# Tai-Wang/Depth-from-Motion

Hardware: NVIDIA H100
Metric: frames/sec (higher is better)
Workload: dtype f32 (bf16x2 split operands, fp32 accumulate)

## Files before the change

### depth_from_motion_b200/csrc/conv_tc.cuh

```cuda
#pragma once
#include <cuda.h>
#include <cuda_bf16.h>

#include <algorithm>
#include <cstdlib>
#include <type_traits>
#include <vector>

#include "common.cuh"
#include "simt_kernels.cuh"
#include "wgmma.cuh"

namespace dfm {

inline uint16_t bf16_rn_bits(float f) {
  uint32_t u;
  memcpy(&u, &f, 4);
  if ((u & 0x7F800000u) == 0x7F800000u) return (uint16_t)(u >> 16);
  u += 0x7FFFu + ((u >> 16) & 1u);
  return (uint16_t)(u >> 16);
}
inline float bf16_bits_to_float(uint16_t b) {
  uint32_t u = (uint32_t)b << 16;
  float f;
  memcpy(&f, &u, 4);
  return f;
}

inline int tc_sm_count() {
  int& cached = per_device<int, 1>();
  if (!cached) cudaDeviceGetAttribute(&cached, cudaDevAttrMultiProcessorCount, cur_device());
  return cached;
}

enum { TC_S1 = 0, TC_S2 = 1, TC_T = 2 };
constexpr int TC_BX = 8, TC_BY = 16;
constexpr int TC_MMA_THREADS = 256;
constexpr int TC_LOAD_THREADS = 256;
constexpr int TC_THREADS = TC_MMA_THREADS + TC_LOAD_THREADS;
constexpr int TC_MAXOPS = 9, TC_MAXBLK = 48;
constexpr int TC_ZERO_TAP = 255;

template <int MODE>
struct TcMode;
template <>
struct TcMode<TC_S1> {
  static constexpr int PXB = 10, PYB = 18, PITCH = 10, ROWS = 186, CG = 32, NSTAGE = 4;
  static constexpr int SLOT_BLOCKS = 1;
  __host__ __device__ static int zo_of(int zi, int dz) { return zi + dz; }
  __host__ __device__ static int zi_first(int zo) { return zo - 1; }
  __host__ __device__ static int zi_last(int zo) { return zo + 1; }
  __host__ __device__ static int ptype(int) { return 0; }
};
template <>
struct TcMode<TC_S2> {
  static constexpr int PXB = 17, PYB = 33, PITCH = 9, ROWS = 620, CG = 16, NSTAGE = 3;
  static constexpr int SLOT_BLOCKS = 1;
  __host__ __device__ static int zo_of(int zi, int dz) { return (zi >> 1) + dz; }
  __host__ __device__ static int zi_first(int zo) { return 2 * zo - 1; }
  __host__ __device__ static int zi_last(int zo) { return 2 * zo + 1; }
  __host__ __device__ static int ptype(int zi) { return zi & 1; }
};
template <>
struct TcMode<TC_T> {
  static constexpr int PXB = 9, PYB = 17, PITCH = 9, ROWS = 154, CG = 32, NSTAGE = 4;
  static constexpr int SLOT_BLOCKS = 4;
  __host__ __device__ static int zo_of(int zi, int dz) { return 2 * zi + dz; }
  __host__ __device__ static int zi_first(int zo) { return zo >> 1; }
  __host__ __device__ static int zi_last(int zo) { return (zo + 1) >> 1; }
  __host__ __device__ static int ptype(int) { return 0; }
};

inline int tc_mode_of(const ConvGeom& g) {
  if (g.transposed) return TC_T;
  if (g.sd == 1 && g.sh == 1 && g.sw == 1 && g.pd == 1 && g.ph == 1 && g.pw == 1) return TC_S1;
  if (g.sd == 2 && g.sh == 2 && g.sw == 2 && g.pd == 1 && g.ph == 1 && g.pw == 1 &&
      g.Di % 2 == 0 && g.Hi % 2 == 0 && g.Wi % 2 == 0)
    return TC_S2;
  return -1;
}
inline bool tc_supported(int Cin, int Cout, int ) {
  if (Cin != 32 && Cin != 64) return false;
  const int ncta = 1024 / Cin;
  return Cout % ncta == 0 && Cout <= 64;
}
inline bool tc_geom_supported(const ConvGeom& g) { return tc_mode_of(g) >= 0; }

struct TcOp {
  uint32_t a_off;
  uint32_t b_off;
  uint32_t b_lbo;
  uint16_t blk0, blk1;
  uint32_t nruns;
  uint32_t runs[3];
};
struct TcBlk {
  int8_t dz;
  uint8_t colblk;
  uint8_t tap;
  uint8_t pad;
};
struct TcProgram {
  int nops;
  uint32_t need;
  TcOp ops[TC_MAXOPS];
  TcBlk blks[TC_MAXBLK];
};

template <int MODE>
inline void tc_build_program(int ptype, int Cin, int ncta, uint32_t* w_cursor, TcProgram* pr) {
  using M = TcMode<MODE>;
  pr->nops = 0;
  pr->need = 0;
  int nb = 0;
  auto add_op = [&](int a_rows, std::vector<TcBlk> blks) {
    TcOp& op = pr->ops[pr->nops++];
    op.a_off = (uint32_t)a_rows * 16;
    op.b_off = *w_cursor;
    op.b_lbo = (uint32_t)blks.size() * ncta * 16;
    op.blk0 = (uint16_t)nb;
    for (TcBlk b : blks) pr->blks[nb++] = b;
    op.blk1 = (uint16_t)nb;
    *w_cursor += (uint32_t)(Cin / 8) * op.b_lbo;
    op.nruns = 0;
    size_t i = 0;
    while (i < blks.size()) {
      size_t e = i + 1;
      auto lin = [&](const TcBlk& b) { return (b.dz + 1) * M::SLOT_BLOCKS + b.colblk; };
      while (e < blks.size() && lin(blks[e]) == lin(blks[i]) + (int)(e - i)) ++e;
      const int nblk = (int)(e - i);
      op.runs[op.nruns++] = (uint32_t)nblk | ((uint32_t)i << 4) | ((uint32_t)lin(blks[i]) << 10);
      for (size_t k = i; k < e; ++k) pr->need |= 1u << (blks[k].dz + 1);
      i = e;
    }
  };
  if (MODE == TC_S1) {
    for (int t = 0; t < 9; ++t) {
      const int dy = t / 3, dx = t % 3;
      add_op(dy * M::PITCH + dx, {TcBlk{-1, 0, (uint8_t)(18 + t), 0}, TcBlk{0, 0, (uint8_t)(9 + t), 0},
                                  TcBlk{1, 0, (uint8_t)t, 0}});
    }
  } else if (MODE == TC_S2) {
    for (int t = 0; t < 9; ++t) {
      const int dy = t / 3, dx = t % 3;
      const int a_rows = (((dx & 1) * 2 + (dy & 1)) * 17 + (dy >> 1)) * M::PITCH + (dx >> 1);
      if (ptype == 0)
        add_op(a_rows, {TcBlk{0, 0, (uint8_t)(9 + t), 0}});
      else
        add_op(a_rows, {TcBlk{0, 0, (uint8_t)(18 + t), 0}, TcBlk{1, 0, (uint8_t)t, 0}});
    }
  } else {
    const int cls_px[4] = {0, 1, 1, 0}, cls_py[4] = {0, 0, 1, 1};
    for (int sh = 0; sh < 4; ++sh) {
      const int sx = sh & 1, sy = sh >> 1;
      std::vector<TcBlk> blks;
      for (int dz = -1; dz <= 1; ++dz) {
        const int kz = dz + 1;
        for (int c = 0; c < 4; ++c) {
          const int px = cls_px[c], py = cls_py[c];
          int kx = -1, ky = -1;
          if (px == 0) { if (!sx) kx = 1; } else kx = sx ? 0 : 2;
          if (py == 0) { if (!sy) ky = 1; } else ky = sy ? 0 : 2;
          const bool real = kx >= 0 && ky >= 0;
          blks.push_back(TcBlk{(int8_t)dz, (uint8_t)c,
                               (uint8_t)(real ? kz * 9 + ky * 3 + kx : TC_ZERO_TAP), 0});
        }
      }
      if (sh == 3) {
        std::vector<TcBlk> real;
        for (const TcBlk& b : blks)
          if (b.tap != TC_ZERO_TAP) real.push_back(b);
        blks = real;
      } else {
        while (!blks.empty() && blks.front().tap == TC_ZERO_TAP) blks.erase(blks.begin());
        while (!blks.empty() && blks.back().tap == TC_ZERO_TAP) blks.pop_back();
      }
      add_op(sy * M::PITCH + sx, blks);
    }
  }
}

struct TcWeights {
  uint8_t* dev = nullptr;
  int Cin = 0, Cout = 0, ncta = 0, nsplit = 0, mode = -1, kslice = 0;
  uint32_t image_bytes = 0, hi_bytes = 0;
  TcProgram prog[2];

  bool ready() const { return dev != nullptr; }
  void release() {
    if (dev) cudaFree(dev);
    dev = nullptr;
  }
  template <int MODE>
  bool build_mode(const float* packed, int cin, int cout, std::string* err, bool ks = false) {
    release();
    mode = MODE;
    Cin = cin;
    Cout = cout;
    kslice = ks ? 1 : 0;
    const int cin_img = ks ? 16 : cin;
    ncta = ks ? cout : 1024 / cin;
    nsplit = ks ? cin / 16 : cout / ncta;
    uint32_t cursor = 0;
    const int ntypes = MODE == TC_S2 ? 2 : 1;
    for (int t = 0; t < ntypes; ++t) tc_build_program<MODE>(t, cin_img, ncta, &cursor, &prog[t]);
    hi_bytes = cursor;
    image_bytes = 2 * hi_bytes;
    std::vector<uint16_t> img((size_t)nsplit * image_bytes / 2);
    const int kch = cin_img / 8;
    for (int s = 0; s < nsplit; ++s)
      for (int t = 0; t < ntypes; ++t)
        for (int o = 0; o < prog[t].nops; ++o) {
          const TcOp& op = prog[t].ops[o];
          const int nblk = op.blk1 - op.blk0;
          for (int kc = 0; kc < kch; ++kc)
            for (int b = 0; b < nblk; ++b)
              for (int j = 0; j < ncta; ++j)
                for (int e = 0; e < 8; ++e) {
                  const int tap = prog[t].blks[op.blk0 + b].tap;
                  if (tap == TC_ZERO_TAP) continue;
                  const int ci = kc * 8 + e + (ks ? s * 16 : 0), co = ks ? j : s * ncta + j;
                  const float w = packed[((size_t)tap * cin + ci) * cout + co];
                  const uint16_t hi = bf16_rn_bits(w);
                  const uint16_t lo = bf16_rn_bits(w - bf16_bits_to_float(hi));
                  const size_t off = (size_t)s * image_bytes / 2 + op.b_off / 2 +
                                     ((size_t)kc * nblk * ncta + (size_t)b * ncta + j) * 8 + e;
                  img[off] = hi;
                  img[off + hi_bytes / 2] = lo;
                }
        }
    if (cudaMalloc(&dev, img.size() * 2) != cudaSuccess ||
        cudaMemcpy(dev, img.data(), img.size() * 2, cudaMemcpyHostToDevice) != cudaSuccess) {
      if (err) *err = "TcWeights: device upload failed";
      release();
      return false;
    }
    return true;
  }
  bool build(const float* packed, int cin, int cout, int m, std::string* err) {
    static const bool no_ks1 = getenv("DFM_NO_KSLICE") != nullptr;
    static const bool ks1 = getenv("DFM_KSLICE_S1") != nullptr;
    if (m == TC_S1) return build_mode<TC_S1>(packed, cin, cout, err,
                                             cin == 64 && cout == 64 && !no_ks1 && ks1);
    if (m == TC_S2) {
      static const bool no_ks = getenv("DFM_NO_KSLICE") != nullptr;
      return build_mode<TC_S2>(packed, cin, cout, err, cout == 64 && !no_ks);
    }
    return build_mode<TC_T>(packed, cin, cout, err);
  }
};

__device__ __forceinline__ uint32_t smem_u32(const void* p) {
  return static_cast<uint32_t>(__cvta_generic_to_shared(p));
}
__device__ __forceinline__ void mbar_init(uint32_t bar, uint32_t count) {
  asm volatile("mbarrier.init.shared::cta.b64 [%0], %1;" ::"r"(bar), "r"(count));
}
__device__ __forceinline__ void mbar_arrive(uint32_t bar) {
  asm volatile("mbarrier.arrive.shared::cta.b64 _, [%0];" ::"r"(bar) : "memory");
}
__device__ __forceinline__ void mbar_wait(uint32_t bar, uint32_t parity, int* err) {
  for (int it = 0; it < (1 << 26); ++it) {
    uint32_t ok;
    asm volatile(
        "{\n\t.reg .pred q;\n\t"
        "mbarrier.try_wait.parity.shared::cta.b64 q, [%1], %2;\n\t"
        "selp.u32 %0, 1, 0, q;\n\t}\n"
        : "=r"(ok)
        : "r"(bar), "r"(parity)
        : "memory");
    if (ok) return;
  }
  *reinterpret_cast<volatile int*>(err) = 1;
  __threadfence_system();
}
__device__ __forceinline__ void mbar_wait_timed(uint32_t bar, uint32_t parity, int* err,
                                                unsigned long long& acc, bool timed) {
  if (!timed) {
    mbar_wait(bar, parity, err);
    return;
  }
  const long long t0 = clock64();
  mbar_wait(bar, parity, err);
  acc += (unsigned long long)(clock64() - t0);
}
__device__ __forceinline__ bool elect_one() {
  uint32_t pred;
  asm volatile(
      "{\n\t.reg .pred p;\n\telect.sync _|p, 0xffffffff;\n\tselp.u32 %0, 1, 0, p;\n\t}\n"
      : "=r"(pred));
  return pred != 0;
}
__device__ __forceinline__ void desc_add(uint64_t& d, uint32_t inc16) {
  asm("{\n\t.reg .b32 lo, hi;\n\tmov.b64 {lo, hi}, %0;\n\tadd.u32 lo, lo, %1;\n\t"
      "mov.b64 %0, {lo, hi};\n\t}\n"
      : "+l"(d)
      : "r"(inc16));
}
__device__ __forceinline__ uint64_t pack64(uint32_t lo, uint32_t hi) {
  return ((uint64_t)hi << 32) | lo;
}
__device__ __forceinline__ void split_store(const float v[8], uint8_t* hi_dst, uint8_t* lo_dst) {
  uint32_t h[4], l[4];
#pragma unroll
  for (int i = 0; i < 4; ++i) {
    const __nv_bfloat162 hh = __floats2bfloat162_rn(v[2 * i], v[2 * i + 1]);
    const float2 hf = __bfloat1622float2(hh);
    const __nv_bfloat162 ll = __floats2bfloat162_rn(v[2 * i] - hf.x, v[2 * i + 1] - hf.y);
    h[i] = *reinterpret_cast<const uint32_t*>(&hh);
    l[i] = *reinterpret_cast<const uint32_t*>(&ll);
  }
  *reinterpret_cast<uint4*>(hi_dst) = make_uint4(h[0], h[1], h[2], h[3]);
  *reinterpret_cast<uint4*>(lo_dst) = make_uint4(l[0], l[1], l[2], l[3]);
}

#ifndef DFM_LD_VARIANT
#define DFM_LD_VARIANT 0
#endif
__device__ __forceinline__ float4 ld_act(const float4* p) {
#if DFM_LD_VARIANT == 1
  return __ldcg(p);
#elif DFM_LD_VARIANT == 2
  float4 v;
  asm volatile("ld.global.nc.L1::no_allocate.L2::256B.v4.f32 {%0,%1,%2,%3}, [%4];"
               : "=f"(v.x), "=f"(v.y), "=f"(v.z), "=f"(v.w) : "l"(p));
  return v;
#elif DFM_LD_VARIANT == 3
  return __ldcs(p);
#elif DFM_LD_VARIANT == 4
  float4 v;
  asm volatile("ld.global.nc.L1::no_allocate.v4.f32 {%0,%1,%2,%3}, [%4];"
               : "=f"(v.x), "=f"(v.y), "=f"(v.z), "=f"(v.w) : "l"(p));
  return v;
#else
  return __ldg(p);
#endif
}

template <int NT>
struct SrcLoader8 {
  static constexpr bool kTma = false;
  Src s;
  int C, H, W;
  static constexpr int BATCH = 6 / NT;
  struct Raw {
    float4 a[NT][2];
  };
  __device__ __forceinline__ void issue(int z, int y, int x, int c0, Raw& r) const {
    const long long inpl = ((long long)y * W + x) * C + c0, plane = (long long)H * W * C;
#pragma unroll
    for (int t = 0; t < NT; ++t) {
      const float* px = s.t[t].x + term_plane(s.t[t], z) * plane + inpl;
      r.a[t][0] = ld_act(reinterpret_cast<const float4*>(px));
      r.a[t][1] = ld_act(reinterpret_cast<const float4*>(px) + 1);
    }
  }
  __device__ __forceinline__ void finish(const Raw& r, int c0, float v[8]) const {
#pragma unroll
    for (int i = 0; i < 8; ++i) v[i] = 0.f;
#pragma unroll
    for (int t = 0; t < NT; ++t) {
      {
        float u[8] = {r.a[t][0].x, r.a[t][0].y, r.a[t][0].z, r.a[t][0].w,
                      r.a[t][1].x, r.a[t][1].y, r.a[t][1].z, r.a[t][1].w};
        if (s.t[t].scale) {
          const float4 s0 = __ldg(reinterpret_cast<const float4*>(s.t[t].scale + c0));
          const float4 s1 = __ldg(reinterpret_cast<const float4*>(s.t[t].scale + c0) + 1);
          const float4 h0 = __ldg(reinterpret_cast<const float4*>(s.t[t].shift + c0));
          const float4 h1 = __ldg(reinterpret_cast<const float4*>(s.t[t].shift + c0) + 1);
          const float sc[8] = {s0.x, s0.y, s0.z, s0.w, s1.x, s1.y, s1.z, s1.w};
          const float sh[8] = {h0.x, h0.y, h0.z, h0.w, h1.x, h1.y, h1.z, h1.w};
#pragma unroll
          for (int i = 0; i < 8; ++i) u[i] = fmaf(u[i], sc[i], sh[i]);
        }
        if (s.t[t].relu) {
#pragma unroll
          for (int i = 0; i < 8; ++i) u[i] = fmaxf(u[i], 0.f);
        }
#pragma unroll
        for (int i = 0; i < 8; ++i) v[i] += u[i];
      }
    }
    if (s.outer_relu) {
#pragma unroll
      for (int i = 0; i < 8; ++i) v[i] = fmaxf(v[i], 0.f);
    }
  }
};

struct WarpLoader8 {
  static constexpr bool kTma = false;
  WarpLoader w;
  static constexpr int BATCH = 1;
  struct Raw {
    float4 t[4][2];
    float wt[4];
  };
  __device__ __forceinline__ void issue(int z, int y, int x, int c0, Raw& r) const {
    c0 += w.first;
    if (c0 < w.C) {
      const float* p = w.cur + ((long long)(y * w.g.step) * w.g.Wf + x * w.g.step) * w.C + c0;
      r.t[0][0] = __ldg(reinterpret_cast<const float4*>(p));
      r.t[0][1] = __ldg(reinterpret_cast<const float4*>(p) + 1);
      r.wt[0] = 1.f;
      r.wt[1] = r.wt[2] = r.wt[3] = 0.f;
      return;
    }
    c0 -= w.C;
    float fx, fy;
    warp_coord(w.g, x, y, __ldg(w.depths + z), fx, fy);
    const Taps t = bilinear_taps(fx, fy, w.g.Hf, w.g.Wf);
#pragma unroll
    for (int k = 0; k < 4; ++k) {
      r.wt[k] = t.w[k];
      if (t.w[k] != 0.f) {
        const float* p = w.prev + (long long)t.off[k] * w.C + c0;
        r.t[k][0] = __ldg(reinterpret_cast<const float4*>(p));
        r.t[k][1] = __ldg(reinterpret_cast<const float4*>(p) + 1);
      }
    }
  }
  __device__ __forceinline__ void finish(const Raw& r, int, float v[8]) const {
#pragma unroll
    for (int i = 0; i < 8; ++i) v[i] = 0.f;
#pragma unroll
    for (int k = 0; k < 4; ++k) {
      if (r.wt[k] != 0.f) {
        v[0] = fmaf(r.wt[k], r.t[k][0].x, v[0]); v[1] = fmaf(r.wt[k], r.t[k][0].y, v[1]);
        v[2] = fmaf(r.wt[k], r.t[k][0].z, v[2]); v[3] = fmaf(r.wt[k], r.t[k][0].w, v[3]);
        v[4] = fmaf(r.wt[k], r.t[k][1].x, v[4]); v[5] = fmaf(r.wt[k], r.t[k][1].y, v[5]);
        v[6] = fmaf(r.wt[k], r.t[k][1].z, v[6]); v[7] = fmaf(r.wt[k], r.t[k][1].w, v[7]);
      }
    }
  }
};

struct TmaLoader8 {
  static constexpr bool kTma = true;
  static constexpr int BATCH = 1;
  CUtensorMap map;
  int nch_total;
  struct Raw {};
  __device__ __forceinline__ void issue(int, int, int, int, Raw&) const {}
  __device__ __forceinline__ void finish(const Raw&, int, float v[8]) const {
#pragma unroll
    for (int i = 0; i < 8; ++i) v[i] = 0.f;
  }
};
constexpr int TMA_S2_CLS = 17 * 9;
constexpr int TMA_S2_CLSR = (2 * TMA_S2_CLS + 7) / 8 * 8;

__device__ __forceinline__ void tma_load_4d(uint32_t dst, const CUtensorMap* map, int c1, int c2,
                                            int c3, uint32_t bar) {
  asm volatile(
      "cp.async.bulk.tensor.4d.shared::cluster.global.tile.mbarrier::complete_tx::bytes "
      "[%0], [%1, {%2, %3, %4, %5}], [%6];" ::"r"(dst),
      "l"(map), "r"(0), "r"(c1), "r"(c2), "r"(c3), "r"(bar)
      : "memory");
}

constexpr int PS_XRUN = 64, PS_WARPS = 4, PS_SEG = 33;
inline size_t presplit_smem_bytes(int C) { return (size_t)PS_WARPS * 4 * (C / 8) * PS_SEG * 16; }
template <int NT>
__global__ void __launch_bounds__(32 * PS_WARPS)
presplit_kernel(const SrcLoader8<NT> ld, int Z, uint4* __restrict__ out) {
  extern __shared__ uint4 ps_sm[];
  const int nch = ld.C >> 3, W = ld.W, H = ld.H, W2 = W >> 1, H2 = H >> 1;
  const int warp = threadIdx.x >> 5, lane = threadIdx.x & 31;
  uint4* sm = ps_sm + (size_t)warp * 4 * nch * PS_SEG;
  const int runs_per_row = (W + PS_XRUN - 1) / PS_XRUN;
  const long long nruns = (long long)Z * H * runs_per_row;
  for (long long r = (long long)blockIdx.x * PS_WARPS + warp; r < nruns;
       r += (long long)gridDim.x * PS_WARPS) {
    const int run = (int)(r % runs_per_row);
    const long long zy = r / runs_per_row;
    const int y = (int)(zy % H), z = (int)(zy / H);
    const int xb = run * PS_XRUN;
#pragma unroll 4
    for (int i = lane; i < PS_XRUN * nch; i += 32) {
      const int xl = i / nch, chunk = i - xl * nch, x = xb + xl;
      if (x < W) {
        typename SrcLoader8<NT>::Raw raw;
        ld.issue(z, y, x, chunk * 8, raw);
        float val[8];
        ld.finish(raw, chunk * 8, val);
        uint4* hi = sm + ((xl & 1) * nch + chunk) * PS_SEG + (xl >> 1);
        split_store(val, reinterpret_cast<uint8_t*>(hi),
                    reinterpret_cast<uint8_t*>(hi + 2 * nch * PS_SEG));
      }
    }
    __syncwarp();
    const int py = y & 1, y2 = y >> 1, x2 = (xb >> 1) + lane;
    for (int seg = 0; seg < 4 * nch; ++seg) {
      const int chunk = seg % nch, px = (seg / nch) & 1, hl = seg / (2 * nch);
      if (2 * x2 + px < W)
        out[((((long long)(z * 2 + hl) * 4 + py * 2 + px) * nch + chunk) * H2 + y2) * W2 + x2] =
            sm[seg * PS_SEG + lane];
    }
    __syncwarp();
  }
}
inline bool presplit_launch(const Src& s, int C, int Z, int H, int W, uint4* out, cudaStream_t st) {
  if ((H | W) & 1) return false;
  const size_t smem = presplit_smem_bytes(C);
  const long long nruns = (long long)Z * H * ((W + PS_XRUN - 1) / PS_XRUN);
  const int blocks = (int)std::min<long long>((nruns + PS_WARPS - 1) / PS_WARPS, 12LL * tc_sm_count());
  auto go = [&](auto kern, auto ld) {
    if (cudaFuncSetAttribute(kern, cudaFuncAttributeMaxDynamicSharedMemorySize, (int)smem) !=
        cudaSuccess)
      return false;
    kern<<<blocks, 32 * PS_WARPS, smem, st>>>(ld, Z, out);
    return cudaGetLastError() == cudaSuccess;
  };
  if (s.n == 1) return go(presplit_kernel<1>, SrcLoader8<1>{s, C, H, W});
  if (s.n == 2) return go(presplit_kernel<2>, SrcLoader8<2>{s, C, H, W});
  return go(presplit_kernel<3>, SrcLoader8<3>{s, C, H, W});
}

inline bool make_presplit_map_s2(CUtensorMap* map, const void* base, int W, int H,
                                 long long slabs, std::string* err) {
  typedef CUresult (*EncodeFn)(CUtensorMap*, CUtensorMapDataType, cuuint32_t, void*,
                               const cuuint64_t*, const cuuint64_t*, const cuuint32_t*,
                               const cuuint32_t*, CUtensorMapInterleave, CUtensorMapSwizzle,
                               CUtensorMapL2promotion, CUtensorMapFloatOOBfill);
  static EncodeFn encode = nullptr;
  if (!encode) {
    void* fn = nullptr;
    cudaDriverEntryPointQueryResult qres;
    if (cudaGetDriverEntryPoint("cuTensorMapEncodeTiled", &fn, cudaEnableDefault, &qres) !=
            cudaSuccess || !fn || qres != cudaDriverEntryPointSuccess) {
      if (err) *err = "cuTensorMapEncodeTiled is not available from this driver";
      return false;
    }
    encode = (EncodeFn)fn;
  }
  const int W2 = W / 2, H2 = H / 2;
  const cuuint64_t dims[4] = {8, (cuuint64_t)W2, (cuuint64_t)H2, (cuuint64_t)slabs};
  const cuuint64_t strides[3] = {16, (cuuint64_t)W2 * 16, (cuuint64_t)H2 * W2 * 16};
  const cuuint32_t box[4] = {8, 9, 17, 2};
  const cuuint32_t estr[4] = {1, 1, 1, 1};
  const CUresult r = encode(map, CU_TENSOR_MAP_DATA_TYPE_UINT16, 4, const_cast<void*>(base), dims,
                            strides, box, estr, CU_TENSOR_MAP_INTERLEAVE_NONE,
                            CU_TENSOR_MAP_SWIZZLE_NONE, CU_TENSOR_MAP_L2_PROMOTION_L2_128B,
                            CU_TENSOR_MAP_FLOAT_OOB_FILL_NONE);
  if (r != CUDA_SUCCESS) {
    if (err) *err = "cuTensorMapEncodeTiled failed with code " + std::to_string((int)r);
    return false;
  }
  return true;
}

struct TcParams {
  const uint8_t* wimg;
  float* out;
  double* stats;
  int Di, Hi, Wi;
  int Do, Ho, Wo, Cout;
  int Mx, My;
  int tiles_x, tiles_y, nsplit;
  int z_unit;
  uint32_t w_bytes, w_hi_bytes;
  int* err;
  unsigned long long* role_cycles;
  const float* addend;
  int zw_lo, zw_hi;
  float zw;
  long long slice_stride;
  int store1;
  int dbg;
};

struct TcItem {
  int x0, y0, split, z_lo, z_hi;
};
struct TcWalk {
  long long cur, end;
  int split;
};
__device__ __forceinline__ TcWalk tc_walk_begin(const TcParams& p) {
  TcWalk w;
  const int per_split = gridDim.x / p.nsplit;
  w.split = blockIdx.x % p.nsplit;
  const int r = blockIdx.x / p.nsplit;
  const long long units_col = p.Do / p.z_unit;
  const long long total = (long long)p.tiles_x * p.tiles_y * units_col;
  w.cur = total * r / per_split;
  w.end = total * (r + 1) / per_split;
  return w;
}
__device__ __forceinline__ bool tc_walk_next(const TcParams& p, TcWalk& w, TcItem& it) {
  if (w.cur >= w.end) return false;
  const long long units_col = p.Do / p.z_unit;
  const int col = (int)(w.cur / units_col);
  const long long u0 = w.cur % units_col;
  const long long u1 = min(units_col, u0 + (w.end - w.cur));
  it.split = w.split;
  it.x0 = (col % p.tiles_x) * TC_BX;
  it.y0 = (col / p.tiles_x) * TC_BY;
  it.z_lo = (int)u0 * p.z_unit;
  it.z_hi = (int)u1 * p.z_unit;
  w.cur += u1 - u0;
  return true;
}

template <int MODE>
struct TcWin;
template <>
struct TcWin<TC_S1> {
  static constexpr int NPL = 3;
  __device__ static int base(int zi) { return zi - 1; }
};
template <>
struct TcWin<TC_S2> {
  static constexpr int NPL = 2;
  __device__ static int base(int zi) { return zi >> 1; }
};
template <>
struct TcWin<TC_T> {
  static constexpr int NPL = 3;
  __device__ static int base(int zi) { return 2 * zi - 1; }
};

template <int MODE, int CIN, int NCTA, class Loader>
__global__ void __launch_bounds__(TC_THREADS, 1) conv_tc_kernel(const __grid_constant__ TcParams p,
                                                                 const __grid_constant__ Loader ld) {
  using M = TcMode<MODE>;
  using Win = TcWin<MODE>;
  constexpr bool TMA = Loader::kTma;
  static_assert(!TMA || MODE == TC_S2, "the TMA loader serves the stride-2 brick only");
  constexpr int CG = M::CG < CIN ? M::CG : CIN;
  constexpr int NCH = CG / 8;
  constexpr int NCG = CIN / CG;
  static_assert(!TMA || NCH == 2, "TMA stride-2 stages hold two 8-channel chunks");
  constexpr uint32_t S2_CLS16 = TMA ? TMA_S2_CLSR : TMA_S2_CLS;
  constexpr uint32_t A_LBO = TMA ? TMA_S2_CLS * 16 : M::ROWS * 16;
  constexpr uint32_t A_SBO = M::PITCH * 16;
  constexpr uint32_t A_HL = TMA ? 4 * TMA_S2_CLSR * 16 : NCH * M::ROWS * 16;
  constexpr uint32_t STAGE_BYTES = 2 * A_HL;
  constexpr uint32_t B_SBO = 128;
  constexpr bool KSLICE = CIN == 16;
  constexpr int NPOS = M::PXB * M::PYB;
  constexpr int LGROUPS = 2;
  constexpr int LG_THREADS = TC_LOAD_THREADS / LGROUPS;
  constexpr int NITEM = (NPOS * NCH + LG_THREADS - 1) / LG_THREADS;
  constexpr int PCOLS = M::SLOT_BLOCKS * NCTA;
  constexpr int NACC = Win::NPL * PCOLS / 2;

  extern __shared__ __align__(1024) uint8_t smem[];
  uint8_t* w_s = smem;
  uint8_t* a_s = smem + p.w_bytes;
  uint64_t* bars = reinterpret_cast<uint64_t*>(a_s + M::NSTAGE * STAGE_BYTES);

  const int tid = threadIdx.x, lane = tid & 31;
  const int warp = __shfl_sync(0xffffffffu, tid >> 5, 0);
  const uint32_t bar0 = smem_u32(bars);
  auto full_a = [&](int s) { return bar0 + 8u * s; };
  auto empty_a = [&](int s) { return bar0 + 8u * (M::NSTAGE + s); };
  const uint32_t w_bar = bar0 + 8u * (2 * M::NSTAGE);
  constexpr int LOAD_WARP0 = TC_MMA_THREADS / 32;

  if (tid == 0) {
    for (int s = 0; s < M::NSTAGE; ++s) {
      mbar_init(full_a(s), TMA ? 1 : LG_THREADS / 32);
      mbar_init(empty_a(s), TC_MMA_THREADS / 32);
    }
    mbar_init(w_bar, 1);
    asm volatile("fence.mbarrier_init.release.cluster;" ::: "memory");
    const int split = blockIdx.x % p.nsplit;
    const uint8_t* src = p.wimg + (size_t)split * p.w_bytes;
    asm volatile("mbarrier.arrive.expect_tx.shared::cta.b64 _, [%0], %1;" ::"r"(w_bar),
                 "r"(p.w_bytes)
                 : "memory");
    constexpr uint32_t CHUNK = 32768;
    for (uint32_t off = 0; off < p.w_bytes; off += CHUNK) {
      const uint32_t n = min(CHUNK, p.w_bytes - off);
      asm volatile(
          "cp.async.bulk.shared::cluster.global.mbarrier::complete_tx::bytes [%0], [%1], %2, [%3];"
          ::"r"(smem_u32(w_s + off)), "l"(src + off), "r"(n), "r"(w_bar)
          : "memory");
    }
  }
  __syncthreads();

  if constexpr (TMA) {
    if (warp == LOAD_WARP0 && lane == 0) {
      constexpr uint32_t STAGE_TX = 8u * 2u * TMA_S2_CLS * 16u;
      uint32_t stage_ctr = 0;
      TcWalk walk = tc_walk_begin(p);
      TcItem it;
      while (tc_walk_next(p, walk, it)) {
        const int zi0 = max(M::zi_first(it.z_lo), 0);
        const int zi1 = min(M::zi_last(it.z_hi - 1), p.Di - 1);
        const int chunk0 = CIN == 16 ? it.split * 2 : 0;
        for (int zi = zi0; zi <= zi1; ++zi) {
#pragma unroll 1
          for (int cg = 0; cg < NCG; ++cg, ++stage_ctr) {
            const int s = stage_ctr % M::NSTAGE;
            mbar_wait(empty_a(s), ((stage_ctr / M::NSTAGE) & 1) ^ 1, p.err);
            asm volatile("mbarrier.arrive.expect_tx.shared::cta.b64 _, [%0], %1;" ::"r"(full_a(s)),
                         "r"(STAGE_TX)
                         : "memory");
            const uint32_t st_addr = smem_u32(a_s + s * STAGE_BYTES);
#pragma unroll
            for (int hl = 0; hl < 2; ++hl) {
#pragma unroll
              for (int cls = 0; cls < 4; ++cls) {
                const int bxp = cls >> 1, byp = cls & 1;
                const int cls_in = (1 - byp) * 2 + (1 - bxp);
                const int slab = ((zi * 2 + hl) * 4 + cls_in) * ld.nch_total + chunk0 + cg * NCH;
                tma_load_4d(st_addr + hl * A_HL + cls * (TMA_S2_CLSR * 16), &ld.map,
                            it.x0 - 1 + bxp, it.y0 - 1 + byp, slab, full_a(s));
              }
            }
          }
        }
      }
    }
  }
  if (TMA && warp >= LOAD_WARP0) {
  } else if (warp >= LOAD_WARP0) {
    const int lw = warp - LOAD_WARP0;
    const int lgrp = lw & (LGROUPS - 1);
    const int lt = (lw / LGROUPS) * 32 + lane;
    const int chunk = lt % NCH;
    uint32_t stage_ctr = 0;
    const bool timed = p.role_cycles != nullptr && lw == 0 && lane == 0;
    unsigned long long t_wait_e = 0;
    const long long t_begin = clock64();
    TcWalk walk = tc_walk_begin(p);
    TcItem it;
    while (tc_walk_next(p, walk, it)) {
      int soff[NITEM], gx[NITEM], gy[NITEM];
      bool inb[NITEM], live[NITEM];
#pragma unroll
      for (int k = 0; k < NITEM; ++k) {
        const int i = lt + k * LG_THREADS;
        live[k] = i < NPOS * NCH;
        const int pos = i / NCH;
        const int bx = pos % M::PXB, by = pos / M::PXB;
        int row;
        if (MODE == TC_S1) {
          gx[k] = it.x0 - 1 + bx;
          gy[k] = it.y0 - 1 + by;
          row = by * M::PITCH + bx;
        } else if (MODE == TC_S2) {
          gx[k] = 2 * it.x0 - 1 + bx;
          gy[k] = 2 * it.y0 - 1 + by;
          row = (((bx & 1) * 2 + (by & 1)) * 17 + (by >> 1)) * M::PITCH + (bx >> 1);
        } else {
          gx[k] = it.x0 + bx;
          gy[k] = it.y0 + by;
          row = by * M::PITCH + bx;
        }
        inb[k] = live[k] && gx[k] >= 0 && gx[k] < p.Wi && gy[k] >= 0 && gy[k] < p.Hi;
        soff[k] = (chunk * M::ROWS + row) * 16;
      }
      const int zi0 = max(M::zi_first(it.z_lo), 0);
      const int zi1 = min(M::zi_last(it.z_hi - 1), p.Di - 1);
      for (int zi = zi0; zi <= zi1; ++zi) {
#pragma unroll 1
        for (int cg = 0; cg < NCG; ++cg, ++stage_ctr) {
          if ((int)(stage_ctr & (LGROUPS - 1)) != lgrp) continue;
          const int s = stage_ctr % M::NSTAGE;
          mbar_wait_timed(empty_a(s), ((stage_ctr / M::NSTAGE) & 1) ^ 1, p.err, t_wait_e, timed);
          uint8_t* st = a_s + s * STAGE_BYTES;
          const int c0 = cg * CG + chunk * 8 + (KSLICE ? it.split * CIN : 0);
          constexpr int LB = Loader::BATCH < NITEM ? Loader::BATCH : NITEM;
          if (!(p.dbg & 1))
#pragma unroll
          for (int k0 = 0; k0 < NITEM; k0 += LB) {
            typename Loader::Raw raw[LB];
#pragma unroll
            for (int b = 0; b < LB; ++b)
              if (k0 + b < NITEM && inb[k0 + b] && !(p.dbg & 16))
                ld.issue(zi, gy[k0 + b], gx[k0 + b], c0, raw[b]);
#pragma unroll
            for (int b = 0; b < LB; ++b) {
              if (k0 + b < NITEM && live[k0 + b]) {
                float v[8];
                if (inb[k0 + b]) {
                  ld.finish(raw[b], c0, v);
                } else {
#pragma unroll
                  for (int i = 0; i < 8; ++i) v[i] = 0.f;
                }
                if (!(p.dbg & 32)) split_store(v, st + soff[k0 + b], st + A_HL + soff[k0 + b]);
                else if (v[0] + v[1] + v[2] + v[3] + v[4] + v[5] + v[6] + v[7] == 1.2345f) st[0] = 1;
              }
            }
          }
          if (!(p.dbg & 8)) asm volatile("fence.proxy.async.shared::cta;" ::: "memory");
          __syncwarp();
          if (lane == 0) mbar_arrive(full_a(s));
        }
      }
    }
    if (timed) {
      unsigned long long* rc = p.role_cycles + (size_t)blockIdx.x * 8;
      rc[3] = (unsigned long long)(clock64() - t_begin);
      rc[4] = t_wait_e;
    }
  } else {
    const int wg = warp >> 2, wq = warp & 3;
    const bool timed = p.role_cycles != nullptr && tid == 0;
    unsigned long long t_wait_a = 0;
    const long long t_begin = clock64();
    mbar_wait(w_bar, 0u, p.err);
    const uint32_t w_base = smem_u32(w_s), a_base = smem_u32(a_s);
    constexpr uint32_t A_LBO16 = A_LBO >> 4, A_HL16 = A_HL >> 4;
    const uint32_t a_desc_hi = A_SBO >> 4;
    const uint32_t b_desc_hi = B_SBO >> 4;
    const uint32_t w_hi16 = p.w_hi_bytes >> 4;
    const uint32_t a_wg16 = (uint32_t)wg * 8u * (A_SBO >> 4);

    float acc[NACC];
#pragma unroll
    for (int i = 0; i < NACC; ++i) acc[i] = 0.f;
    constexpr int NST = KSLICE ? 1 : NCTA / 4;
    float ssum[NST], ssq[NST];
#pragma unroll
    for (int i = 0; i < NST; ++i) ssum[i] = ssq[i] = 0.f;

    const int xr = lane >> 2, cq = lane & 3;
    auto flush_stats = [&](int split) {
      if (KSLICE || !p.stats) return;
#pragma unroll
      for (int k = 0; k < NST; ++k) {
        double a = ssum[k], b = ssq[k];
#pragma unroll
        for (int o = 4; o < 32; o <<= 1) {
          a += __shfl_xor_sync(0xffffffffu, a, o);
          b += __shfl_xor_sync(0xffffffffu, b, o);
        }
        if (lane < 4) {
          const int ch = split * NCTA + 8 * (k >> 1) + 2 * lane + (k & 1);
          atomicAdd(p.stats + 2 * ch, a);
          atomicAdd(p.stats + 2 * ch + 1, b);
        }
        ssum[k] = ssq[k] = 0.f;
      }
    };
    auto emit = [&](const TcItem& it, auto jc, int zo) {
      constexpr int J = decltype(jc)::value;
      if (zo < it.z_lo || zo >= it.z_hi) return;
#pragma unroll
      for (int cb = 0; cb < M::SLOT_BLOCKS; ++cb) {
        const float* r = acc + (J * PCOLS + cb * NCTA) / 2;
#pragma unroll
        for (int rr = 0; rr < 2; ++rr) {
          const int mx = it.x0 + xr, my = it.y0 + 8 * wg + 2 * wq + rr;
          if (mx >= p.Mx || my >= p.My) continue;
          int xo = mx, yo = my;
          if (MODE == TC_T) {
            xo = 2 * mx + ((cb == 1 || cb == 2) ? 1 : 0);
            yo = 2 * my + (cb >= 2 ? 1 : 0);
          }
          const long long vox = ((long long)zo * p.Ho + yo) * p.Wo + xo;
          if (p.store1) {
            if (cq == 0) p.out[vox] = r[2 * rr];
            continue;
          }
          const int ch_base = (KSLICE ? 0 : it.split * NCTA) + 2 * cq;
          const float wz = (zo >= p.zw_lo && zo < p.zw_hi) ? p.zw : 1.f;
#pragma unroll
          for (int j = 0; j < NCTA / 8; ++j) {
            float v0 = r[4 * j + 2 * rr], v1 = r[4 * j + 2 * rr + 1];
            const int ch = ch_base + 8 * j;
            if (p.addend) {
              const int cls = zo == 0 ? 0 : (zo == p.Do - 1 ? 2 : 1);
              const float2 a2 = __ldg(reinterpret_cast<const float2*>(
                  p.addend + (((long long)cls * p.Ho + yo) * p.Wo + xo) * p.Cout + ch));
              v0 += a2.x;
              v1 += a2.y;
            }
            *reinterpret_cast<float2*>(p.out + (KSLICE ? it.split * p.slice_stride : 0) +
                                       vox * p.Cout + ch) = make_float2(v0, v1);
            if constexpr (!KSLICE) {
              if (p.stats) {
                ssum[2 * j] = fmaf(wz, v0, ssum[2 * j]);
                ssq[2 * j] = fmaf(wz * v0, v0, ssq[2 * j]);
                ssum[2 * j + 1] = fmaf(wz, v1, ssum[2 * j + 1]);
                ssq[2 * j + 1] = fmaf(wz * v1, v1, ssq[2 * j + 1]);
              }
            }
          }
        }
      }
    };
    auto shift = [&](auto shc) {
      constexpr int SH = decltype(shc)::value * PCOLS / 2;
#pragma unroll
      for (int i = 0; i < NACC; ++i) acc[i] = i + SH < NACC ? acc[i + SH] : 0.f;
    };

    uint32_t stage_ctr = 0;
    TcWalk walk = tc_walk_begin(p);
    TcItem it;
    while (tc_walk_next(p, walk, it)) {
      const int zi0 = max(M::zi_first(it.z_lo), 0);
      const int zi1 = min(M::zi_last(it.z_hi - 1), p.Di - 1);
      for (int zi = zi0; zi <= zi1; ++zi) {
#pragma unroll 1
        for (int cg = 0; cg < NCG; ++cg, ++stage_ctr) {
          const int s = stage_ctr % M::NSTAGE;
          mbar_wait_timed(full_a(s), (stage_ctr / M::NSTAGE) & 1, p.err, t_wait_a, timed);
          __syncwarp();
          const uint32_t a_lo_stage =
              ((((a_base + s * STAGE_BYTES) >> 4) & 0x3FFF) + a_wg16) | (A_LBO16 << 16);
          wgmma_fence();
          if constexpr (MODE == TC_S1) {
            constexpr uint32_t B_LBO16 = 3 * NCTA;
            constexpr uint32_t TAP16 = (CIN / 8) * B_LBO16;
            constexpr int NKS = CG / 16;
            const uint32_t b_lo0 = ((w_base >> 4) & 0x3FFF) + (uint32_t)(cg * NCH) * B_LBO16 +
                                   (B_LBO16 << 16);
            uint64_t da[NKS][2], db[NKS][2];
#pragma unroll
            for (int ks = 0; ks < NKS; ++ks) {
              da[ks][0] = pack64(a_lo_stage + 2 * ks * A_LBO16, a_desc_hi);
              da[ks][1] = pack64(a_lo_stage + 2 * ks * A_LBO16 + A_HL16, a_desc_hi);
              const uint32_t bl = b_lo0 + 2 * ks * B_LBO16;
              db[ks][0] = pack64(bl, b_desc_hi);
              db[ks][1] = pack64(bl + w_hi16, b_desc_hi);
            }
#pragma unroll 1
            for (int tap = 0; tap < 9; ++tap) {
#pragma unroll
              for (int ks = 0; ks < NKS; ++ks) {
                wgmma_bf16<3 * NCTA>(acc, da[ks][0], db[ks][0]);
                wgmma_bf16<3 * NCTA>(acc, da[ks][1], db[ks][0]);
                wgmma_bf16<3 * NCTA>(acc, da[ks][0], db[ks][1]);
              }
              const uint32_t ainc = (tap == 2 || tap == 5) ? (uint32_t)(M::PITCH - 2) : 1u;
#pragma unroll
              for (int ks = 0; ks < NKS; ++ks) {
                desc_add(da[ks][0], ainc);
                desc_add(da[ks][1], ainc);
                desc_add(db[ks][0], TAP16);
                desc_add(db[ks][1], TAP16);
              }
            }
          }
          if constexpr (MODE == TC_S2) {
            constexpr uint32_t KCH16 = CIN / 8;
            const uint32_t odd = (uint32_t)zi & 1u;
            auto run = [&](auto nbc) {
              constexpr uint32_t NB = decltype(nbc)::value;
              constexpr uint32_t b_lbo16 = NB * NCTA;
              constexpr uint32_t tap16 = KCH16 * b_lbo16;
              const uint32_t b_lo0 = ((w_base >> 4) & 0x3FFF) + (NB == 2 ? 9u * KCH16 * NCTA : 0u) +
                                     (uint32_t)(cg * NCH) * b_lbo16 + (b_lbo16 << 16);
              uint64_t dbh = pack64(b_lo0, b_desc_hi);
              uint64_t dbl = pack64(b_lo0 + w_hi16, b_desc_hi);
#pragma unroll
              for (int tap = 0; tap < 9; ++tap) {
                const int dy = tap / 3, dx = tap % 3;
                const uint32_t a16 = (uint32_t)(((dx & 1) * 2 + (dy & 1)) * S2_CLS16 +
                                                (dy >> 1) * M::PITCH + (dx >> 1));
                const uint64_t dah = pack64(a_lo_stage + a16, a_desc_hi);
                const uint64_t dal = pack64(a_lo_stage + a16 + A_HL16, a_desc_hi);
                wgmma_bf16<NB * NCTA>(acc, dah, dbh);
                wgmma_bf16<NB * NCTA>(acc, dal, dbh);
                wgmma_bf16<NB * NCTA>(acc, dah, dbl);
                desc_add(dbh, tap16);
                desc_add(dbl, tap16);
              }
            };
            if (odd) run(std::integral_constant<uint32_t, 2>());
            else run(std::integral_constant<uint32_t, 1>());
          }
          if constexpr (MODE == TC_T) {
            constexpr uint32_t KCH16 = CIN / 8;
            constexpr uint32_t NB[4] = {12u, 10u, 10u, 3u};
            constexpr uint32_t LIN0[4] = {0u, 1u, 2u, 2u};
            uint32_t b_img16 = (w_base >> 4) & 0x3FFF;
#pragma unroll
            for (int sh = 0; sh < 4; ++sh) {
              const uint32_t b_lbo16 = NB[sh] * NCTA;
              const uint32_t a16 = (uint32_t)((sh >> 1) * M::PITCH + (sh & 1));
#pragma unroll
              for (int ks = 0; ks < CG / 16; ++ks) {
                const uint32_t alo = a_lo_stage + a16 + 2 * ks * A_LBO16;
                const uint64_t dah = pack64(alo, a_desc_hi);
                const uint64_t dal = pack64(alo + A_HL16, a_desc_hi);
                const uint32_t blo = b_img16 + (uint32_t)(cg * NCH + 2 * ks) * b_lbo16 +
                                     (b_lbo16 << 16);
                auto mma3 = [&](float* d, uint32_t bl, auto nc) {
                  constexpr int N = decltype(nc)::value;
                  const uint64_t dbh = pack64(bl, b_desc_hi);
                  const uint64_t dbl = pack64(bl + w_hi16, b_desc_hi);
                  wgmma_bf16<N>(d, dah, dbh);
                  wgmma_bf16<N>(d, dal, dbh);
                  wgmma_bf16<N>(d, dah, dbl);
                };
                if (sh == 0) {
                  mma3(acc, blo, std::integral_constant<int, 12 * NCTA>());
                } else if (sh == 1) {
                  mma3(acc + NCTA / 2, blo, std::integral_constant<int, 10 * NCTA>());
                } else if (sh == 2) {
                  mma3(acc + NCTA, blo, std::integral_constant<int, 10 * NCTA>());
                } else {
#pragma unroll
                  for (uint32_t k = 0; k < 3; ++k)
                    mma3(acc + (LIN0[3] + k * 4) * (NCTA / 2), blo + k * NCTA,
                         std::integral_constant<int, NCTA>());
                }
              }
              b_img16 += KCH16 * b_lbo16;
            }
          }
          wgmma_commit();
          wgmma_wait<0>();
          __syncwarp();
          if (lane == 0) mbar_arrive(empty_a(s));
        }
        if constexpr (MODE == TC_S1) {
          emit(it, std::integral_constant<int, 0>(), zi - 1);
          shift(std::integral_constant<int, 1>());
        } else if constexpr (MODE == TC_S2) {
          if (zi & 1) {
            emit(it, std::integral_constant<int, 0>(), zi >> 1);
            shift(std::integral_constant<int, 1>());
          }
        } else {
          emit(it, std::integral_constant<int, 0>(), 2 * zi - 1);
          emit(it, std::integral_constant<int, 1>(), 2 * zi);
          shift(std::integral_constant<int, 2>());
        }
      }
      const int zb = Win::base(zi1 + 1);
      emit(it, std::integral_constant<int, 0>(), zb);
      emit(it, std::integral_constant<int, 1>(), zb + 1);
      if constexpr (Win::NPL > 2) emit(it, std::integral_constant<int, 2>(), zb + 2);
#pragma unroll
      for (int i = 0; i < NACC; ++i) acc[i] = 0.f;
      flush_stats(it.split);
    }
    if (timed) {
      unsigned long long* rc = p.role_cycles + (size_t)blockIdx.x * 8;
      rc[0] = (unsigned long long)(clock64() - t_begin);
      rc[1] = t_wait_a;
    }
  }
}

struct TcErrFlag {
  int* host = nullptr;
  int* dev = nullptr;
  int* get() {
    if (!host) {
      if (cudaHostAlloc(&host, sizeof(int), cudaHostAllocMapped | cudaHostAllocPortable) !=
          cudaSuccess) {
        host = nullptr;
        cudaGetLastError();
        return nullptr;
      }
      *host = 0;
      cudaHostGetDevicePointer(&dev, host, 0);
    }
    return dev;
  }
};
inline TcErrFlag& tc_err_flag() {
  static TcErrFlag f;
  return f;
}
inline int tc_consume_error() {
  TcErrFlag& f = tc_err_flag();
  if (!f.host) return 0;
  const int h = *reinterpret_cast<volatile int*>(f.host);
  if (h) *reinterpret_cast<volatile int*>(f.host) = 0;
  return h;
}

__global__ void __launch_bounds__(256)
kslice_reduce_kernel(const float* __restrict__ part, int nsl, long long V, long long HW,
                     float* __restrict__ out, double* __restrict__ stats, int zw_lo, int zw_hi,
                     float zw) {
  __shared__ double sh[2][16][64];
  const int q = threadIdx.x & 15, r = threadIdx.x >> 4;
  double s[4] = {0, 0, 0, 0}, ss[4] = {0, 0, 0, 0};
  const long long w0 = (long long)zw_lo * HW, w1 = (long long)zw_hi * HW;
  for (long long v = (long long)blockIdx.x * 16 + r; v < V; v += (long long)gridDim.x * 16) {
    float4 a = __ldg(reinterpret_cast<const float4*>(part + v * 64) + q);
    for (int k = 1; k < nsl; ++k) {
      const float4 b = __ldg(reinterpret_cast<const float4*>(part + ((long long)k * V + v) * 64) + q);
      a.x += b.x; a.y += b.y; a.z += b.z; a.w += b.w;
    }
    reinterpret_cast<float4*>(out + v * 64)[q] = a;
    if (stats) {
      const double wgt = (v >= w0 && v < w1) ? (double)zw : 1.0;
      s[0] += wgt * a.x; ss[0] += wgt * (double)a.x * a.x;
      s[1] += wgt * a.y; ss[1] += wgt * (double)a.y * a.y;
      s[2] += wgt * a.z; ss[2] += wgt * (double)a.z * a.z;
      s[3] += wgt * a.w; ss[3] += wgt * (double)a.w * a.w;
    }
  }
  if (!stats) return;
#pragma unroll
  for (int i = 0; i < 4; ++i) {
    sh[0][r][4 * q + i] = s[i];
    sh[1][r][4 * q + i] = ss[i];
  }
  __syncthreads();
  if (threadIdx.x < 128) {
    const int c = threadIdx.x & 63, which = threadIdx.x >> 6;
    double t = 0.0;
    for (int k = 0; k < 16; ++k) t += sh[which][k][c];
    atomicAdd(stats + 2 * c + which, t);
  }
}
struct TcScratch {
  float* p = nullptr;
  size_t n = 0;
  float* get(size_t count) {
    if (n >= count) return p;
    if (p) cudaFree(p);
    p = nullptr;
    n = 0;
    if (cudaMalloc(&p, count * sizeof(float)) != cudaSuccess) return nullptr;
    n = count;
    return p;
  }
};
inline TcScratch& tc_kslice_scratch() { return per_device<TcScratch>(); }

struct TcOpts {
  int store1 = 0;
  const float* addend = nullptr;
  int zw_lo = 0, zw_hi = 0;
  float zw = 1.f;
  long long slice_stride = 0;
};
template <int MODE, int CIN, int NCTA, class Loader>
bool tc_launch(const Loader& ld, const TcWeights& w, float* out, double* stats,
               const ConvGeom& g, cudaStream_t st, std::string* err, TcOpts opt = TcOpts()) {
  using M = TcMode<MODE>;
  constexpr int CG = M::CG < CIN ? M::CG : CIN;
  constexpr size_t STAGE_BYTES = Loader::kTma ? (size_t)2 * 4 * TMA_S2_CLSR * 16
                                              : (size_t)2 * (CG / 8) * M::ROWS * 16;
  const size_t smem = w.image_bytes + M::NSTAGE * STAGE_BYTES + (2 * M::NSTAGE + 1) * 8;
  auto kern = conv_tc_kernel<MODE, CIN, NCTA, Loader>;
  struct AttrTag { size_t v = 0; };
  static AttrTag attr_dev[kMaxDevices];
  size_t& attr_smem = attr_dev[cur_device()].v;
  if (smem > attr_smem) {
    if (smem > 232448 ||
        cudaFuncSetAttribute(kern, cudaFuncAttributeMaxDynamicSharedMemorySize, (int)smem) !=
            cudaSuccess) {
      if (err) *err = "conv_tc: cannot reserve " + std::to_string(smem) + " B of shared memory";
      return false;
    }
    attr_smem = smem;
  }
  const int sms = tc_sm_count();
  TcParams p{};
  p.wimg = w.dev;
  p.out = out;
  p.stats = stats;
  p.store1 = opt.store1;
  p.slice_stride = opt.slice_stride;
  p.addend = opt.addend;
  p.zw_lo = opt.zw_lo;
  p.zw_hi = opt.zw_hi;
  p.zw = opt.zw;
  p.Di = g.Di; p.Hi = g.Hi; p.Wi = g.Wi;
  p.Do = g.Do; p.Ho = g.Ho; p.Wo = g.Wo;
  p.Cout = g.Cout;
  p.Mx = MODE == TC_T ? g.Wi : g.Wo;
  p.My = MODE == TC_T ? g.Hi : g.Ho;
  p.tiles_x = (p.Mx + TC_BX - 1) / TC_BX;
  p.tiles_y = (p.My + TC_BY - 1) / TC_BY;
  p.nsplit = w.nsplit;
  p.w_bytes = w.image_bytes;
  p.w_hi_bytes = w.hi_bytes;
  p.z_unit = MODE == TC_T ? 2 : 1;
  const long long cols = (long long)p.tiles_x * p.tiles_y;
  const long long units = cols * (g.Do / p.z_unit);
  int per_split = std::max(1, sms / p.nsplit);
  per_split = (int)std::min<long long>(per_split, units);
  const int grid = per_split * p.nsplit;
  p.err = tc_err_flag().get();
  static const bool role_dbg = getenv("DFM_TC_ROLE_CYCLES") != nullptr;
  static const int dbg_flags = getenv("DFM_TC_DEBUG") ? atoi(getenv("DFM_TC_DEBUG")) : 0;
  p.dbg = dbg_flags;
  static unsigned long long* role_buf = nullptr;
  if (role_dbg) {
    if (!role_buf) cudaMalloc(&role_buf, 1024 * 8 * sizeof(unsigned long long));
    cudaMemsetAsync(role_buf, 0, 1024 * 8 * sizeof(unsigned long long), st);
    p.role_cycles = role_buf;
  }
  kern<<<grid, TC_THREADS, smem, st>>>(p, ld);
  if (role_dbg) {
    cudaStreamSynchronize(st);
    std::vector<unsigned long long> h((size_t)grid * 8);
    cudaMemcpy(h.data(), role_buf, h.size() * 8, cudaMemcpyDeviceToHost);
    double a[8] = {0};
    for (int b = 0; b < grid; ++b)
      for (int k = 0; k < 8; ++k) a[k] += (double)h[(size_t)b * 8 + k] / grid;
    fprintf(stderr,
            "[tc mode=%d cin=%d ncta=%d grid=%d cols=%lld Do=%d] mma+epilogue: total %.0f "
            "wait_full_a %.0f | load: total %.0f wait_empty_a %.0f\n",
            MODE, CIN, NCTA, grid, cols, g.Do, a[0], a[1], a[3], a[4]);
  }
  const cudaError_t e = cudaGetLastError();
  if (e != cudaSuccess) {
    if (err) *err = std::string("conv_tc launch: ") + cudaGetErrorString(e);
    return false;
  }
  return true;
}

template <class Loader>
bool tc_dispatch(const Loader& ld, const TcWeights& w, float* out, double* stats,
                 const ConvGeom& g, cudaStream_t st, std::string* err, TcOpts opt = TcOpts()) {
  const int mode = tc_mode_of(g);
  if (mode != w.mode) {
    if (err) *err = "conv_tc: weight image was built for a different conv mode";
    return false;
  }
  if (w.kslice) {
    if ((mode != TC_S2 && mode != TC_S1) || g.Cout != 64 || opt.addend || opt.store1) {
      if (err) *err = "conv_tc: K-slice weights are for plain convs with 64 outputs";
      return false;
    }
    const long long V = (long long)g.Do * g.Ho * g.Wo;
    float* part = tc_kslice_scratch().get((size_t)w.nsplit * V * 64);
    if (!part) {
      if (err) *err = "conv_tc: cannot allocate the K-slice scratch";
      return false;
    }
    TcOpts o2 = opt;
    o2.slice_stride = V * 64;
    bool launched = false;
    if constexpr (Loader::kTma) {
      if (mode == TC_S2) launched = tc_launch<TC_S2, 16, 64, Loader>(ld, w, part, nullptr, g, st, err, o2);
      else if (err) *err = "conv_tc: the TMA loader serves stride-2 convs only";
    } else {
      launched = mode == TC_S2
                     ? tc_launch<TC_S2, 16, 64, Loader>(ld, w, part, nullptr, g, st, err, o2)
                     : tc_launch<TC_S1, 16, 64, Loader>(ld, w, part, nullptr, g, st, err, o2);
    }
    if (!launched) return false;
    const int blocks = (int)std::min<long long>(8LL * tc_sm_count(), (V + 15) / 16);
    kslice_reduce_kernel<<<blocks, 256, 0, st>>>(part, w.nsplit, V, (long long)g.Ho * g.Wo, out,
                                                 stats, opt.zw_lo, opt.zw_hi, opt.zw);
    if (cudaGetLastError() != cudaSuccess) {
      if (err) *err = "conv_tc: kslice_reduce_kernel launch failed";
      return false;
    }
    return true;
  }
  if constexpr (Loader::kTma) {
    if (err) *err = "conv_tc: the TMA loader serves the K-slice stride-2 convs only";
    return false;
  } else {
#define TC_CASE(MD, CI, NC) \
  if (mode == MD && g.Cin == CI) \
    return tc_launch<MD, CI, NC, Loader>(ld, w, out, stats, g, st, err, opt)
  TC_CASE(TC_S1, 32, 32);
  TC_CASE(TC_S1, 64, 16);
  TC_CASE(TC_S2, 32, 32);
  TC_CASE(TC_S2, 64, 16);
  TC_CASE(TC_T, 64, 16);
#undef TC_CASE
  if (err) *err = "conv_tc: unsupported (mode, Cin)";
  return false;
  }
}

inline bool tc_conv_src(const Src& s, const TcWeights& w, float* out, double* stats,
                        const ConvGeom& g, cudaStream_t st, std::string* err,
                        TcOpts opt = TcOpts()) {
  if (s.n == 1) {
    SrcLoader8<1> ld{s, g.Cin, g.Hi, g.Wi};
    return tc_dispatch(ld, w, out, stats, g, st, err, opt);
  }
  if (s.n == 2) {
    SrcLoader8<2> ld{s, g.Cin, g.Hi, g.Wi};
    return tc_dispatch(ld, w, out, stats, g, st, err, opt);
  }
  SrcLoader8<3> ld{s, g.Cin, g.Hi, g.Wi};
  return tc_dispatch(ld, w, out, stats, g, st, err, opt);
}
inline bool tc_conv_presplit(const uint4* ps, int channels, const TcWeights& w, float* out,
                             double* stats, const ConvGeom& g, cudaStream_t st, std::string* err,
                             TcOpts opt = TcOpts()) {
  if (tc_mode_of(g) != TC_S2 || !w.kslice || channels != g.Cin) {
    if (err) *err = "conv_tc: the TMA loader serves the K-slice stride-2 convs only";
    return false;
  }
  TmaLoader8 ld;
  ld.nch_total = channels / 8;
  if (!make_presplit_map_s2(&ld.map, ps, g.Wi, g.Hi, (long long)g.Di * 2 * 4 * ld.nch_total, err))
    return false;
  return tc_dispatch(ld, w, out, stats, g, st, err, opt);
}
inline bool tc_conv_warp(const WarpLoader& wl, const TcWeights& w, float* out, double* stats,
                         const ConvGeom& g, cudaStream_t st, std::string* err,
                         TcOpts opt = TcOpts()) {
  if (tc_mode_of(g) != TC_S1) {
    if (err) *err = "conv_tc: the warp loader feeds stride-1 convs only";
    return false;
  }
  WarpLoader8 ld{wl};
  if (g.Cin == 32)
    return tc_launch<TC_S1, 32, 32, WarpLoader8>(ld, w, out, stats, g, st, err, opt);
  if (g.Cin == 64)
    return tc_launch<TC_S1, 64, 16, WarpLoader8>(ld, w, out, stats, g, st, err, opt);
  if (err) *err = "conv_tc: unsupported Cin";
  return false;
}

}
```

Measured before the change: 101.2.

## Batch presplit loads per lane and shrink TMA conv block to one loader warp

The presplit kernel is specialised on channel count, with each lane owning one fixed 8-channel chunk. Per-term scale and shift are hoisted into registers, and several pixels' float4 loads are batched before the affine/relu/split math, replacing the generic loader. This aims to raise memory-level parallelism and cut index arithmetic. Separately, the TMA-loader conv kernel now launches with the MMA threads plus a single loader warp, reducing block size and register pressure. That assumes the kernel body only uses one load warp in TMA mode, which cannot be checked from the visible code.

```diff
diff --git a/depth_from_motion_b200/csrc/conv_tc.cuh b/depth_from_motion_b200/csrc/conv_tc.cuh
--- a/depth_from_motion_b200/csrc/conv_tc.cuh
+++ b/depth_from_motion_b200/csrc/conv_tc.cuh
@@ -38,6 +38,9 @@
 constexpr int TC_MMA_THREADS = 256;
 constexpr int TC_LOAD_THREADS = 256;
 constexpr int TC_THREADS = TC_MMA_THREADS + TC_LOAD_THREADS;
+constexpr int TC_TMA_THREADS = TC_MMA_THREADS + 32;
+template <class Loader>
+constexpr int tc_threads() { return Loader::kTma ? TC_TMA_THREADS : TC_THREADS; }
 constexpr int TC_MAXOPS = 9, TC_MAXBLK = 48;
 constexpr int TC_ZERO_TAP = 255;
 
@@ -461,40 +464,105 @@
 
 constexpr int PS_XRUN = 64, PS_WARPS = 4, PS_SEG = 33;
 inline size_t presplit_smem_bytes(int C) { return (size_t)PS_WARPS * 4 * (C / 8) * PS_SEG * 16; }
-template <int NT>
+template <int NT, int NCH>
 __global__ void __launch_bounds__(32 * PS_WARPS)
-presplit_kernel(const SrcLoader8<NT> ld, int Z, uint4* __restrict__ out) {
+presplit_kernel(const Src s, int Z, int H, int W, uint4* __restrict__ out) {
+  static_assert(32 % NCH == 0, "a lane keeps one chunk");
+  constexpr int C = NCH * 8, XSTEP = 32 / NCH, ITEMS = PS_XRUN / XSTEP;
+  constexpr int PS_BATCH = NT == 1 ? 8 : 4;
   extern __shared__ uint4 ps_sm[];
-  const int nch = ld.C >> 3, W = ld.W, H = ld.H, W2 = W >> 1, H2 = H >> 1;
+  const int W2 = W >> 1, H2 = H >> 1;
   const int warp = threadIdx.x >> 5, lane = threadIdx.x & 31;
-  uint4* sm = ps_sm + (size_t)warp * 4 * nch * PS_SEG;
+  const int chunk = lane % NCH, xl0 = lane / NCH;
+  uint4* sm = ps_sm + (size_t)warp * 4 * NCH * PS_SEG;
+  float sc[NT][8], sh[NT][8];
+#pragma unroll
+  for (int t = 0; t < NT; ++t) {
+#pragma unroll
+    for (int i = 0; i < 8; ++i) {
+      sc[t][i] = 1.f;
+      sh[t][i] = 0.f;
+    }
+    if (s.t[t].scale) {
+      const float4* sp = reinterpret_cast<const float4*>(s.t[t].scale + chunk * 8);
+      const float4* hp = reinterpret_cast<const float4*>(s.t[t].shift + chunk * 8);
+      const float4 s0 = __ldg(sp), s1 = __ldg(sp + 1), h0 = __ldg(hp), h1 = __ldg(hp + 1);
+      const float a[8] = {s0.x, s0.y, s0.z, s0.w, s1.x, s1.y, s1.z, s1.w};
+      const float b[8] = {h0.x, h0.y, h0.z, h0.w, h1.x, h1.y, h1.z, h1.w};
+#pragma unroll
+      for (int i = 0; i < 8; ++i) {
+        sc[t][i] = a[i];
+        sh[t][i] = b[i];
+      }
+    }
+  }
   const int runs_per_row = (W + PS_XRUN - 1) / PS_XRUN;
   const long long nruns = (long long)Z * H * runs_per_row;
+  const long long plane = (long long)H * W * C;
   for (long long r = (long long)blockIdx.x * PS_WARPS + warp; r < nruns;
        r += (long long)gridDim.x * PS_WARPS) {
     const int run = (int)(r % runs_per_row);
     const long long zy = r / runs_per_row;
     const int y = (int)(zy % H), z = (int)(zy / H);
     const int xb = run * PS_XRUN;
-#pragma unroll 4
-    for (int i = lane; i < PS_XRUN * nch; i += 32) {
-      const int xl = i / nch, chunk = i - xl * nch, x = xb + xl;
-      if (x < W) {
-        typename SrcLoader8<NT>::Raw raw;
-        ld.issue(z, y, x, chunk * 8, raw);
-        float val[8];
-        ld.finish(raw, chunk * 8, val);
-        uint4* hi = sm + ((xl & 1) * nch + chunk) * PS_SEG + (xl >> 1);
-        split_store(val, reinterpret_cast<uint8_t*>(hi),
-                    reinterpret_cast<uint8_t*>(hi + 2 * nch * PS_SEG));
+    const float* base[NT];
+#pragma unroll
+    for (int t = 0; t < NT; ++t)
+      base[t] = s.t[t].x + term_plane(s.t[t], z) * plane + ((long long)y * W + xb) * C + chunk * 8;
+#pragma unroll
+    for (int k0 = 0; k0 < ITEMS; k0 += PS_BATCH) {
+      float4 raw[PS_BATCH][NT][2];
+#pragma unroll
+      for (int b = 0; b < PS_BATCH; ++b) {
+        const int xl = xl0 + (k0 + b) * XSTEP;
+        if (xb + xl < W) {
+#pragma unroll
+          for (int t = 0; t < NT; ++t) {
+            const float4* px = reinterpret_cast<const float4*>(base[t] + xl * C);
+            raw[b][t][0] = __ldg(px);
+            raw[b][t][1] = __ldg(px + 1);
+          }
+        }
+      }
+#pragma unroll
+      for (int b = 0; b < PS_BATCH; ++b) {
+        const int xl = xl0 + (k0 + b) * XSTEP;
+        if (xb + xl < W) {
+          float v[8];
+#pragma unroll
+          for (int i = 0; i < 8; ++i) v[i] = 0.f;
+#pragma unroll
+          for (int t = 0; t < NT; ++t) {
+            float u[8] = {raw[b][t][0].x, raw[b][t][0].y, raw[b][t][0].z, raw[b][t][0].w,
+                          raw[b][t][1].x, raw[b][t][1].y, raw[b][t][1].z, raw[b][t][1].w};
+            if (s.t[t].scale) {
+#pragma unroll
+              for (int i = 0; i < 8; ++i) u[i] = fmaf(u[i], sc[t][i], sh[t][i]);
+            }
+            if (s.t[t].relu) {
+#pragma unroll
+              for (int i = 0; i < 8; ++i) u[i] = fmaxf(u[i], 0.f);
+            }
+#pragma unroll
+            for (int i = 0; i < 8; ++i) v[i] += u[i];
+          }
+          if (s.outer_relu) {
+#pragma unroll
+            for (int i = 0; i < 8; ++i) v[i] = fmaxf(v[i], 0.f);
+          }
+          uint4* hi = sm + ((xl & 1) * NCH + chunk) * PS_SEG + (xl >> 1);
+          split_store(v, reinterpret_cast<uint8_t*>(hi),
+                      reinterpret_cast<uint8_t*>(hi + 2 * NCH * PS_SEG));
+        }
       }
     }
     __syncwarp();
     const int py = y & 1, y2 = y >> 1, x2 = (xb >> 1) + lane;
-    for (int seg = 0; seg < 4 * nch; ++seg) {
-      const int chunk = seg % nch, px = (seg / nch) & 1, hl = seg / (2 * nch);
+#pragma unroll
+    for (int seg = 0; seg < 4 * NCH; ++seg) {
+      const int ch = seg % NCH, px = (seg / NCH) & 1, hl = seg / (2 * NCH);
       if (2 * x2 + px < W)
-        out[((((long long)(z * 2 + hl) * 4 + py * 2 + px) * nch + chunk) * H2 + y2) * W2 + x2] =
+        out[((((long long)(z * 2 + hl) * 4 + py * 2 + px) * NCH + ch) * H2 + y2) * W2 + x2] =
             sm[seg * PS_SEG + lane];
     }
     __syncwarp();
@@ -502,19 +570,25 @@
 }
 inline bool presplit_launch(const Src& s, int C, int Z, int H, int W, uint4* out, cudaStream_t st) {
   if ((H | W) & 1) return false;
+  if (C != 32 && C != 64) return false;
   const size_t smem = presplit_smem_bytes(C);
   const long long nruns = (long long)Z * H * ((W + PS_XRUN - 1) / PS_XRUN);
   const int blocks = (int)std::min<long long>((nruns + PS_WARPS - 1) / PS_WARPS, 12LL * tc_sm_count());
-  auto go = [&](auto kern, auto ld) {
+  auto go = [&](auto kern) {
     if (cudaFuncSetAttribute(kern, cudaFuncAttributeMaxDynamicSharedMemorySize, (int)smem) !=
         cudaSuccess)
       return false;
-    kern<<<blocks, 32 * PS_WARPS, smem, st>>>(ld, Z, out);
+    kern<<<blocks, 32 * PS_WARPS, smem, st>>>(s, Z, H, W, out);
     return cudaGetLastError() == cudaSuccess;
   };
-  if (s.n == 1) return go(presplit_kernel<1>, SrcLoader8<1>{s, C, H, W});
-  if (s.n == 2) return go(presplit_kernel<2>, SrcLoader8<2>{s, C, H, W});
-  return go(presplit_kernel<3>, SrcLoader8<3>{s, C, H, W});
+  if (C == 32) {
+    if (s.n == 1) return go(presplit_kernel<1, 4>);
+    if (s.n == 2) return go(presplit_kernel<2, 4>);
+    return go(presplit_kernel<3, 4>);
+  }
+  if (s.n == 1) return go(presplit_kernel<1, 8>);
+  if (s.n == 2) return go(presplit_kernel<2, 8>);
+  return go(presplit_kernel<3, 8>);
 }
 
 inline bool make_presplit_map_s2(CUtensorMap* map, const void* base, int W, int H,
@@ -622,7 +696,7 @@
 };
 
 template <int MODE, int CIN, int NCTA, class Loader>
-__global__ void __launch_bounds__(TC_THREADS, 1) conv_tc_kernel(const __grid_constant__ TcParams p,
+__global__ void __launch_bounds__(tc_threads<Loader>(), 1) conv_tc_kernel(const __grid_constant__ TcParams p,
                                                                  const __grid_constant__ Loader ld) {
   using M = TcMode<MODE>;
   using Win = TcWin<MODE>;
@@ -1190,7 +1264,7 @@
     cudaMemsetAsync(role_buf, 0, 1024 * 8 * sizeof(unsigned long long), st);
     p.role_cycles = role_buf;
   }
-  kern<<<grid, TC_THREADS, smem, st>>>(p, ld);
+  kern<<<grid, tc_threads<Loader>(), smem, st>>>(p, ld);
   if (role_dbg) {
     cudaStreamSynchronize(st);
     std::vector<unsigned long long> h((size_t)grid * 8);
```

Result: faster. 104.0 (median of 6 runs) (+2.8%).
